# DiltheyLab/HLA-LA

Hardware: AMD Instinct MI355X
Metric: paired reads/sec aligned to PRG graph (higher is better)
Workload: dtype int32

## Files before the change

hla-la_amd/csrc/kernel_dp.hip:

```cpp
#include "batch.h"
#include "../../include/hlala_gpu.h"

namespace hlala {

enum { K_DIAG = 0, K_GGAP = 1, K_SGAP = 2, K_HOP = 3, K_JUMP = 4 };
enum { M_D = 0, M_GG = 1, M_SG = 2 };
enum { PH_IDLE = 0, PH_RUN, PH_SELECT, PH_BT, PH_EXPAND, PH_DONE };

constexpr u64 HKEY_EMPTY = ~0ull;
#ifndef HLALA_DP_PROFILE_LOG2
#define HLALA_DP_PROFILE_LOG2 18
#endif
#ifndef HLALA_EARLY_GEN_MAX
#define HLALA_EARLY_GEN_MAX 0xFFFFFE
#endif
constexpr int DP_EARLY_GEN_MAX = HLALA_EARLY_GEN_MAX;
constexpr int EXT_PENDING = 0x7FFFFFFF;
constexpr int DP_BT_STEPS_PER_TRIP = 32;

#ifndef HLALA_DP_TAIL_THREADS
#define HLALA_DP_TAIL_THREADS 128
#endif
constexpr int DP_TAIL_THREADS = HLALA_DP_TAIL_THREADS;
#ifndef HLALA_DP_TINY_WAVES
#define HLALA_DP_TINY_WAVES 4
#endif
#ifndef HLALA_DP_WIDE_THREADS
#define HLALA_DP_WIDE_THREADS 64
#endif
#ifndef HLALA_DP_BROAD_THREADS
#define HLALA_DP_BROAD_THREADS HLALA_DP_TAIL_THREADS
#endif
#ifndef HLALA_DP_LARGE_THREADS
#define HLALA_DP_LARGE_THREADS HLALA_DP_TAIL_THREADS
#endif
#ifndef HLALA_DP_HUGE_THREADS
#define HLALA_DP_HUGE_THREADS HLALA_DP_TAIL_THREADS
#endif
struct DpTiny  { static constexpr bool JF = false; static constexpr int THREADS = 64, WAVES = HLALA_DP_TINY_WAVES, GW = 16, WCAP = 16,   HC = 32,   IBITS = 4,  CELLS = 2048,     EARLY = 4096,     IMPCAP = 64,   COMPLETED = 256,          STEPS = 1024;     typedef u32 Best; typedef short Slot; typedef unsigned char ImpIdx; static constexpr bool IN_MEMORY = false; };
#ifndef HLALA_DP_TINYJF_WAVES
#define HLALA_DP_TINYJF_WAVES 4
#endif
struct DpTinyJF : DpTiny { static constexpr bool JF = true; static constexpr int WAVES = HLALA_DP_TINYJF_WAVES; };
struct DpMid   { static constexpr bool JF = false; static constexpr int THREADS = 64, WAVES = 4, GW = 32, WCAP = 32,   HC = 128,  IBITS = 5,  CELLS = 4096,     EARLY = 8192,     IMPCAP = 256,  COMPLETED = 512,          STEPS = 2048;     typedef u32 Best; typedef short Slot; typedef unsigned short ImpIdx; static constexpr bool IN_MEMORY = false; };
struct DpSmall { static constexpr bool JF = false; static constexpr int THREADS = 64, WAVES = 5, GW = 64, WCAP = 64,   HC = 128,  IBITS = 7,  CELLS = DP_CELLS, EARLY = DP_CELLS, IMPCAP = 2048, COMPLETED = DP_COMPLETED, STEPS = DP_STEPS; typedef u32 Best; typedef short Slot; typedef unsigned short ImpIdx; static constexpr bool IN_MEMORY = false; };
struct DpWide  { static constexpr bool JF = false; static constexpr int THREADS = HLALA_DP_WIDE_THREADS, WAVES = 2, GW = HLALA_DP_WIDE_THREADS, WCAP = 256,  HC = 512,  IBITS = 8,  CELLS = DP_CELLS, EARLY = DP_CELLS, IMPCAP = 2048, COMPLETED = DP_COMPLETED, STEPS = DP_STEPS; typedef u32 Best; typedef short Slot; typedef unsigned short ImpIdx; static constexpr bool IN_MEMORY = false; };
struct DpBroad { static constexpr bool JF = false; static constexpr int THREADS = HLALA_DP_BROAD_THREADS, WAVES = 1, GW = HLALA_DP_BROAD_THREADS, WCAP = 512,  HC = 1024, IBITS = 9,  CELLS = DP_CELLS_LARGE, EARLY = DP_CELLS_LARGE, IMPCAP = 4096, COMPLETED = DP_COMPLETED_LARGE, STEPS = DP_STEPS; typedef u32 Best; typedef int Slot; typedef unsigned short ImpIdx; static constexpr bool IN_MEMORY = false; };
struct DpLarge { static constexpr bool JF = false; static constexpr int THREADS = HLALA_DP_LARGE_THREADS, WAVES = 1, GW = HLALA_DP_LARGE_THREADS, WCAP = 1024, HC = 2048, IBITS = 10, CELLS = DP_CELLS_LARGE, EARLY = DP_CELLS_LARGE, IMPCAP = 4096, COMPLETED = DP_COMPLETED_LARGE, STEPS = DP_STEPS; typedef u32 Best; typedef int Slot; typedef unsigned short ImpIdx; static constexpr bool IN_MEMORY = false; };

struct DpHuge  { static constexpr bool JF = false; static constexpr int THREADS = HLALA_DP_HUGE_THREADS, WAVES = 1, GW = HLALA_DP_HUGE_THREADS, WCAP = 8192, HC = 16384, IBITS = 13, CELLS = 131072, EARLY = 131072, IMPCAP = 8192, COMPLETED = 65536, STEPS = DP_STEPS; typedef u64 Best; typedef int Slot; typedef unsigned short ImpIdx; static constexpr bool IN_MEMORY = true; };
#ifndef HLALA_DP_SORT_SCRATCH
#define HLALA_DP_SORT_SCRATCH 4096
#endif
constexpr int DP_SORT_SCRATCH = HLALA_DP_SORT_SCRATCH;

struct DpState {
    int itemIdx;
    int item, rOff, seqLen, start_seq, startLevel, startNode;
    int d, b1, b2, n1, n2, nCells, nCompleted, curMax, firstMaxSlot, lastInc, earlyInit, itersRun, diagonals;
    int earlyMaxNat;
    u32 cellsEvaluated;
    int endSlot, endScore, nSteps, nCols;
    int have, sb, se, err;
    int isAlias;
    int needTier;
};

template <bool SMALL> struct TlistT { typedef unsigned short type; };
template <> struct TlistT<true> { typedef unsigned char type; };

template <class C>
struct __align__(16) DpLdsT {
    u64 hkey[C::HC];
    typename C::Best hbest[3][C::HC];
    typename TlistT<(C::HC <= 256)>::type tlist[C::HC];
    u64 fkey[2][C::WCAP];
    typename C::Slot fslot[2][C::WCAP];
    short fD[2][C::WCAP], fG[2][C::WCAP], fS[2][C::WCAP];
    typename C::Slot tes[C::HC];
    unsigned char timp[C::HC];
    typename C::ImpIdx hq[C::HC];
    int nNew, nImp, nKeepF, err, nCompletedAdd;
    int chunkNext, chunkEnd;
    int jumpMet;
    int nTa;
    int nextPhase;
    int btSlot, btM, btX, btY, btGuard, btDone;
    DpState st;
    u64 accCalls, accIters, accCells, accEdges;
#ifdef HLALA_DP_TIMING
    long long tPh[16];
#endif
#ifdef HLALA_DP_PROFILE
    long long pfStart; int pfSlow, pfImp, pfPre, pfMaxNT, pfMaxF; long long pfPh[16];
#endif
};

struct __align__(16) CellRec { u64 key; short sc[4]; u32 bt[3]; u32 pad; };

template <class C>
struct DpSlabT {
    char* base;
    static constexpr size_t O_CELL      = 0;
    static constexpr size_t O_EARLY_KEY = O_CELL + (size_t)C::CELLS * 32;
    static constexpr size_t O_STEP_XY   = O_EARLY_KEY + (size_t)C::EARLY * 8;
    static constexpr size_t O_IMP_KEY   = O_STEP_XY + (size_t)C::STEPS * 8;
    static constexpr size_t O_IMP_NEW   = O_IMP_KEY + (size_t)C::IMPCAP * 8;
    static constexpr size_t O_IMP_BT    = O_IMP_NEW + (size_t)C::IMPCAP * 8;
    static constexpr size_t O_STEP_BT   = O_IMP_BT + (size_t)C::IMPCAP * 12;
    static constexpr size_t O_EARLY_VAL = O_STEP_BT + (size_t)C::STEPS * 4;
    static constexpr size_t O_COMPLETED = O_EARLY_VAL + (size_t)C::EARLY * 4;
    static constexpr size_t O_IMP_SLOT  = O_COMPLETED + (size_t)C::COMPLETED * 4;
    static constexpr size_t O_IMP_MASK  = O_IMP_SLOT + (size_t)C::IMPCAP * 4;
    static constexpr size_t O_TIE_SLOT  = O_IMP_MASK + (size_t)C::IMPCAP * 4;
    static constexpr size_t O_TIE_KEY   = (O_TIE_SLOT + (size_t)C::COMPLETED * 4 + 7) & ~(size_t)7;
    static constexpr size_t O_EARLY_GEN = O_TIE_KEY + (size_t)C::COMPLETED * 8;
    static constexpr size_t O_SORT_SPILL = (O_EARLY_GEN + 8 + 15) & ~(size_t)15;
    static constexpr size_t BYTES       = (O_SORT_SPILL + (C::IN_MEMORY ? (size_t)C::WCAP * 16 : 0) + 255) & ~(size_t)255;
    __device__ __forceinline__ CellRec* cell() const { return (CellRec*)(base + O_CELL); }
    __device__ __forceinline__ u64* early_key() const { return (u64*)(base + O_EARLY_KEY); }
    __device__ __forceinline__ u32* step_bt() const { return (u32*)(base + O_STEP_BT); }
    __device__ __forceinline__ u64* step_xy() const { return (u64*)(base + O_STEP_XY); }
    __device__ __forceinline__ u64* imp_key() const { return (u64*)(base + O_IMP_KEY); }
    __device__ __forceinline__ u32* imp_bt() const { return (u32*)(base + O_IMP_BT); }
    __device__ __forceinline__ short* imp_new() const { return (short*)(base + O_IMP_NEW); }
    __device__ __forceinline__ int* early_val() const { return (int*)(base + O_EARLY_VAL); }
    __device__ __forceinline__ int* completed() const { return (int*)(base + O_COMPLETED); }
    __device__ __forceinline__ int* imp_slot() const { return (int*)(base + O_IMP_SLOT); }
    __device__ __forceinline__ int* imp_mask() const { return (int*)(base + O_IMP_MASK); }
    __device__ __forceinline__ int* tie_slot() const { return (int*)(base + O_TIE_SLOT); }
    __device__ __forceinline__ u64* tie_key() const { return (u64*)(base + O_TIE_KEY); }
    __device__ __forceinline__ int* early_gen() const { return (int*)(base + O_EARLY_GEN); }
    __device__ __forceinline__ u64* sort_spill() const { return (u64*)(base + O_SORT_SPILL); }
};

template <class C>
__host__ __device__ inline size_t dp_slab_bytes() { return DpSlabT<C>::BYTES; }
template <class C>
__host__ __device__ inline size_t dp_inmemory_bytes() { return ((sizeof(DpLdsT<C>) + 255) & ~(size_t)255) + DpSlabT<C>::BYTES; }

template <int GW> __device__ __forceinline__ int grp_lane() { return (int)(threadIdx.x & (GW - 1)); }
template <int GW> __device__ __forceinline__ int grp_base() { return (int)(threadIdx.x & 63 & ~(GW - 1)); }

#define HLALA_ROW_ALLREDUCE(v, OP)                                                          \
    do {                                                                                    \
        int t_;                                                                             \
        t_ = __builtin_amdgcn_update_dpp(v, v, 0xB1, 0xF, 0xF, false); v = OP(v, t_);        \
        t_ = __builtin_amdgcn_update_dpp(v, v, 0x4E, 0xF, 0xF, false); v = OP(v, t_);        \
        t_ = __builtin_amdgcn_update_dpp(v, v, 0x141, 0xF, 0xF, false); v = OP(v, t_);           \
        t_ = __builtin_amdgcn_update_dpp(v, v, 0x140, 0xF, 0xF, false); v = OP(v, t_);                \
    } while(0)

__device__ __forceinline__ void blk_barrier()
{
    __builtin_amdgcn_fence(__ATOMIC_RELEASE, "workgroup"); __builtin_amdgcn_s_barrier(); __builtin_amdgcn_fence(__ATOMIC_ACQUIRE, "workgroup");
}
template <int GW> struct BlkX { static constexpr int NW = GW / 64; };
template <int GW> __device__ __forceinline__ int* blk_words() { __shared__ int x[BlkX<GW>::NW > 0 ? 2 * BlkX<GW>::NW : 2]; return x; }

template <int GW> __device__ __forceinline__ int grp_max_i32(int v)
{
    if(GW == 64) return wave_max_i32(v);
    if constexpr (GW > 64) {
        const int w = wave_max_i32(v); int* x = blk_words<GW>();
        if(lane_id() == 0) x[threadIdx.x >> 6] = w;
        blk_barrier();
        int r = x[0];
#pragma unroll
        for(int i = 1; i < BlkX<GW>::NW; i++) r = op_max_(r, x[i]);
        blk_barrier();
        return r;
    } else {
    HLALA_ROW_ALLREDUCE(v, op_max_);
    if(GW == 32) v = op_max_(v, __shfl_xor(v, 16));
    return v;
    }
}
template <int GW> __device__ __forceinline__ int grp_sum_i32(int v)
{
    if(GW == 64) return wave_sum_i32(v);
    if constexpr (GW > 64) {
        const int w = wave_sum_i32(v); int* x = blk_words<GW>();
        if(lane_id() == 0) x[threadIdx.x >> 6] = w;
        blk_barrier();
        int r = x[0];
#pragma unroll
        for(int i = 1; i < BlkX<GW>::NW; i++) r += x[i];
        blk_barrier();
        return r;
    } else {
    HLALA_ROW_ALLREDUCE(v, op_add_);
    if(GW == 32) v = op_add_(v, __shfl_xor(v, 16));
    return v;
    }
}
template <int GW> __device__ __forceinline__ u64 grp_min_u64(u64 v)
{
    if(GW == 64) return wave_min_u64(v);
    int hi = (int)(~(u32)(v >> 32) ^ 0x80000000u);
    int mh = grp_max_i32<GW>(hi);
    int lo = (hi == mh) ? (int)(~(u32)v ^ 0x80000000u) : (int)0x80000000;
    int ml = grp_max_i32<GW>(lo);
    return ((u64)(~((u32)mh ^ 0x80000000u)) << 32) | (u64)(~((u32)ml ^ 0x80000000u));
// ... 168 lines not shown
#pragma nounroll
    for(int probe = 0; probe < C::HC; probe++) {
        u64 old = atomicCAS(&S.hkey[h], HKEY_EMPTY, key);
        if(old == HKEY_EMPTY || old == key) { typename C::Best v; pack_best<C>(v, score, order); atomicMax(&S.hbest[mat][h], v); return true; }
        h = (h + 1) & (C::HC - 1);
    }
    return false;
}

template <class C>
__device__ inline u32 dp_probe(DpLdsT<C>& S, u64 key, u32 h)
{
#pragma nounroll
    for(int probe = 1; probe < C::HC; probe++) {
        h = (h + 1) & (C::HC - 1);
        u64 old = atomicCAS(&S.hkey[h], HKEY_EMPTY, key);
        if(old == HKEY_EMPTY || old == key) return h;
    }
    return (u32)C::HC;
}
template <class C>
__device__ inline u32 dp_probe(DpLdsT<C>& S, u64 key, u32 h, bool& claimed)
{
#pragma nounroll
    for(int probe = 1; probe < C::HC; probe++) {
        h = (h + 1) & (C::HC - 1);
        u64 old = atomicCAS(&S.hkey[h], HKEY_EMPTY, key);
        if(old == HKEY_EMPTY) claimed = true;
        if(old == HKEY_EMPTY || old == key) return h;
    }
    return (u32)C::HC;
}

template <class C> __device__ __forceinline__ u32 early_hash(u64 k) { return (C::EARLY > 8192 ? hash_mix(k) : hash64(k)) & (u32)(C::EARLY - 1); }

__device__ __forceinline__ u64 early_word(int gen, u64 key) { return ((u64)(u32)gen << 40) | (key & 0xFFFFFFFFFFull); }

template <class C>
__device__ inline int early_lookup(const DpSlabT<C>& sl, int gen, u64 key)
{
    u32 h = early_hash<C>(key);
    const u64 w = early_word(gen, key);
    for(int probe = 0; probe < C::EARLY; probe++) {
        u64 cur = __hip_atomic_load(&sl.early_key()[h], __ATOMIC_RELAXED, __HIP_MEMORY_SCOPE_AGENT);
        if(cur == w) return __hip_atomic_load(&sl.early_val()[h], __ATOMIC_RELAXED, __HIP_MEMORY_SCOPE_AGENT);
        if((int)(cur >> 40) != gen) return -1;
        h = (h + 1) & (C::EARLY - 1);
    }
    return -1;
}
template <class C>
__device__ inline bool early_insert(const DpSlabT<C>& sl, int gen, u64 key, int slot)
{
    u32 h = early_hash<C>(key);
    const u64 w = early_word(gen, key);
    for(int probe = 0; probe < C::EARLY; probe++) {
        u64 cur = __hip_atomic_load(&sl.early_key()[h], __ATOMIC_RELAXED, __HIP_MEMORY_SCOPE_AGENT);
        while((int)(cur >> 40) != gen) {
            const u64 old = atomicCAS(&sl.early_key()[h], cur, w);
            if(old == cur) { cur = w; break; }
            cur = old;
        }
        if(cur == w) { __hip_atomic_store(&sl.early_val()[h], slot, __ATOMIC_RELAXED, __HIP_MEMORY_SCOPE_AGENT); return true; }
        h = (h + 1) & (C::EARLY - 1);
    }
    return false;
}

__device__ inline int dec_len(int v) { int n = 1; while(v >= 10) { v /= 10; n++; } return n; }
__device__ inline int pow10i(int n) { int p = 1; while(n-- > 0) p *= 10; return p; }
__device__ __forceinline__ int dec_len_cmp(int v)
{
    return 1 + (v >= 10) + (v >= 100) + (v >= 1000) + (v >= 10000) + (v >= 100000) + (v >= 1000000) + (v >= 10000000) + (v >= 100000000) + (v >= 1000000000);
}
__device__ __forceinline__ u32 pow10_u32(int k)
{
    u32 p = (k & 1) ? 10u : 1u;
    if(k & 2) p *= 100u;
    if(k & 4) p *= 10000u;
    if(k & 8) p *= 100000000u;
    return p;
}
__device__ __forceinline__ int xz_part(int a, int b)
{
    if(a == b) return 0;
    const int la = dec_len_cmp(a), lb = dec_len_cmp(b);
    u64 A = (u64)(u32)a, Bv = (u64)(u32)b;
    if(la < lb) A *= (u64)pow10_u32(lb - la); else if(lb < la) Bv *= (u64)pow10_u32(la - lb);
    if(A != Bv) return A < Bv ? -1 : 1;
    return la < lb ? -1 : 1;
}
__device__ __forceinline__ bool xz_less(int x1, int z1, int x2, int z2)
{
    const int c = xz_part(x1, x2);
    if(c) return c < 0;
    return xz_part(z1, z2) < 0;
}

__device__ inline u64 xz_key(int x, int z)
{
    const int lx = dec_len(x), lz = dec_len(z);
    u64 k = 0; int n = 0;
    for(int i = 0; i < lx; i++, n++) k = k * 12 + (u64)(2 + (x / pow10i(lx - 1 - i)) % 10);
    k = k * 12 + 1; n++;
    for(int i = 0; i < lz && n < 14; i++, n++) k = k * 12 + (u64)(2 + (z / pow10i(lz - 1 - i)) % 10);
    for(; n < 14; n++) k *= 12;
    return k;
}

struct __align__(16) DpItem { int item, rOff, seqLen, start_seq, startLevel, startNode, pad0, pad1; };

#ifndef HLALA_DP_SIDE_TIER
#define HLALA_DP_SIDE_TIER 3
#endif
constexpr int DP_SIDE_TIER = HLALA_DP_SIDE_TIER;
constexpr int DP_LAST_TIER = 6;
constexpr int DP_POOL_TIER = DP_SIDE_TIER > 4 ? DP_SIDE_TIER : 4;
constexpr int DP_POOL_MAX = 8;
__device__ __forceinline__ int tier_for_frontier(int n) { return n <= DpMid::WCAP ? 1 : (n <= DpSmall::WCAP ? 2 : (n <= DpWide::WCAP ? 3 : (n <= DpBroad::WCAP ? 4 : (n <= DpLarge::WCAP ? 5 : 6)))); }
__device__ __forceinline__ int tier_for_targets(int n) { return n <= (DpMid::HC * 3) / 4 ? 1 : (n <= (DpSmall::HC * 3) / 4 ? 2 : (n <= (DpWide::HC * 3) / 4 ? 3 : (n <= (DpBroad::HC * 3) / 4 ? 4 : (n <= (DpLarge::HC * 3) / 4 ? 5 : 6)))); }

#define DP_FAIL(code) do { if(gl == 0 && S.err == 0) S.err = (code); } while(0)

template <class C, class DG>
__device__ inline int dp_begin(DpLdsT<C>& S, const DpSlabT<C>& sl, const DG& G, const DpItem& it, int itemIdx)
{
    constexpr int GW = C::GW;
    const int gl = grp_lane<GW>();
    for(int i = gl; i < C::HC; i += GW) { S.hkey[i] = HKEY_EMPTY; S.hbest[0][i] = 0; S.hbest[1][i] = 0; S.hbest[2][i] = 0; }
    if(gl == 0) {
        DpState& st = S.st;
        st.itemIdx = itemIdx;
        st.item = it.item; st.rOff = it.rOff; st.seqLen = it.seqLen; st.start_seq = it.start_seq; st.startLevel = it.startLevel; st.startNode = it.startNode;
        st.diagonals = it.seqLen + G.L - 1;
        st.d = 1; st.b1 = 0; st.b2 = 1; st.n1 = 1; st.n2 = 0; st.nCells = 1; st.nCompleted = 0;
        st.curMax = 0; st.firstMaxSlot = 0; st.lastInc = 0; st.earlyInit = 0; st.earlyMaxNat = -1; st.itersRun = 0;
        st.cellsEvaluated = 0;
        st.endSlot = -1; st.endScore = 0; st.nSteps = 0; st.nCols = 0;
        st.have = 0; st.sb = 0; st.se = -1; st.err = 0; st.needTier = 0; st.isAlias = 0;
        S.err = 0; S.nTa = 0; S.jumpMet = 0;
#ifdef HLALA_DP_PROFILE
        S.pfStart = clock64(); S.pfSlow = 0; S.pfImp = 0; S.pfPre = 0; S.pfMaxNT = 0; S.pfMaxF = 0; for(int i = 0; i < 16; i++) S.pfPh[i] = 0;
#endif
        CellRec c0; c0.key = mk_key(it.startLevel, it.start_seq, it.startNode);
        c0.sc[0] = 0; c0.sc[1] = (short)DP_NEG; c0.sc[2] = (short)DP_NEG; c0.sc[3] = 0; c0.bt[0] = 0; c0.bt[1] = 0; c0.bt[2] = 0; c0.pad = 0;
        sl.cell()[0] = c0;
        S.fkey[0][0] = mk_key(it.startLevel, it.start_seq, it.startNode); S.fslot[0][0] = 0;
        S.fD[0][0] = 0; S.fG[0][0] = (short)DP_NEG; S.fS[0][0] = (short)DP_NEG;
    }
    DSYNC();
    return PH_RUN;
}

template <class C, class DG>
__device__ inline int dp_iterate(DpLdsT<C>& S, const DpSlabT<C>& sl, const DG& G, const int4* nrec, const uint8_t* readBases, const bool fwd, int& edgesAcc, u64* sortScratch)
{
    constexpr int GW = C::GW;
    const int gl = grp_lane<GW>();
    DpState& st = S.st;
    const int dir = fwd ? 1 : -1;
    const int seqLen = guni<GW>(st.seqLen);
    const int max_levelI = G.L - 1, max_seqI = seqLen;
    const int limitY = fwd ? seqLen : 0;
    const int d = guni<GW>(st.d);
    const int n1 = guni<GW>(st.n1), n2 = guni<GW>(st.n2);
    const int b1 = guni<GW>(st.b1), b2 = guni<GW>(st.b2), bn = b2;
    const int lastInc0 = guni<GW>(st.lastInc), diagonals = guni<GW>(st.diagonals);
    const uint8_t* seqp = readBases + guni<GW>(st.rOff);

    if(d > diagonals || (d - lastInc0) > 40) return PH_SELECT;
    if(n1 == 0 && n2 == 0) {
        int last = lastInc0 + 40; if(last > diagonals) last = diagonals;
        if(gl == 0) st.itersRun = last;
        DSYNC();
        return PH_SELECT;
    }
    if(d > 60000) { if(gl == 0) { st.itersRun = d; st.err = __LINE__; } DSYNC(); return PH_DONE; }

#if defined(HLALA_DP_TIMING)
    long long tq0 = clock64();
#define DP_TQ(i) do { __builtin_amdgcn_s_waitcnt(0); long long t_ = clock64(); if(gl == 0) S.tPh[i] += t_ - tq0; tq0 = t_; } while(0)
#elif defined(HLALA_DP_PROFILE)
    long long tq0 = clock64();
#define DP_TQ(i) do { __builtin_amdgcn_s_waitcnt(0); long long t_ = clock64(); if(gl == 0) S.pfPh[i] += t_ - tq0; tq0 = t_; } while(0)
#else
#define DP_TQ(i) do { } while(0)
#endif
    const int* eoff = fwd ? G.out_off : G.in_off; const int* eto = fwd ? G.out_to : G.in_from; const uint8_t* elab = fwd ? G.out_label : G.in_label;
    const int* joff = fwd ? G.jf_off : G.jb_off; const int* jnode = fwd ? G.jf_node : G.jb_node; const int* jlvl = fwd ? G.jf_lvl : G.jb_lvl;
    const uint8_t* eprk = fwd ? G.out_prank : G.in_prank; const uint8_t* jprk = fwd ? G.jf_prank : G.jb_prank;
    int edges = 0;
    const int nMax = n1 > n2 ? n1 : n2;
    constexpr bool APPEND = (GW >= 64) && (C::WCAP > 64);
    typedef typename TlistT<(C::HC <= 256)>::type TlT;
    int nTa = 0;
    auto append = [&](const bool claimed, const u32 h) {
        if constexpr (APPEND && GW == 64) {
            const u64 m = __ballot(claimed);
            if(claimed) S.tlist[nTa + (int)__builtin_amdgcn_mbcnt_hi((u32)(m >> 32), __builtin_amdgcn_mbcnt_lo((u32)m, 0u))] = (TlT)h;
            nTa += __popcll(m);
        } else if constexpr (APPEND) {
            const u64 m = __ballot(claimed);
            if(m) {
                int base = 0;
                if(lane_id() == 0) base = atomicAdd(&S.nTa, (int)__popcll(m));
                base = __builtin_amdgcn_readfirstlane(base);
                const int pos = base + (int)__builtin_amdgcn_mbcnt_hi((u32)(m >> 32), __builtin_amdgcn_mbcnt_lo((u32)m, 0u));
                if(claimed && pos < C::HC) S.tlist[pos] = (TlT)h;
            }
        }
    };
    for(int i = gl; i < nMax; i += GW) {
        const bool hasA = i < n2, hasB = i < n1;
        u64 pkA = hasA ? S.fkey[b2][i] : 0, pkB = hasB ? S.fkey[b1][i] : 0;
        const int pxA = key_x(pkA), pyA = key_y(pkA), nodeA = key_node(pkA);
        const int pxB = key_x(pkB), pyB = key_y(pkB), nodeB = key_node(pkB);
        const int nxA = pxA + dir, nyA = pyA + dir;
        const bool doA = hasA && !(nxA > max_levelI || nyA > max_seqI || nxA < 0 || nyA < 0);
        const int pDA = hasA ? (int)S.fD[b2][i] : 0;
        const int pD = hasB ? (int)S.fD[b1][i] : 0, pG = hasB ? (int)S.fG[b1][i] : 0, pS = hasB ? (int)S.fS[b1][i] : 0;
        int4 ra0 = make_int4(0, 0, 0, 0), ra1 = ra0, rb0 = ra0, rb1 = ra0; unsigned char rc = 0;
        if(doA) { ra0 = nrec[2 * (size_t)nodeA]; ra1 = nrec[2 * (size_t)nodeA + 1]; rc = fwd ? seqp[pyA] : seqp[pyA - 1]; }
        if(hasB) { rb0 = nrec[2 * (size_t)nodeB]; rb1 = nrec[2 * (size_t)nodeB + 1]; }
        const int a0 = ra0.x, degA = ra0.y & 0xFFFF, tnA0 = ra0.z, tnA1 = ra0.w;
        const unsigned char labA0 = (unsigned char)(ra1.w & 0xFF), labA1 = (unsigned char)((ra1.w >> 8) & 0xFF);
        const int rkA1 = (ra1.w >> 16) & 1, rkB1 = (rb1.w >> 16) & 1;
        const int e0 = rb0.x, degB = rb0.y & 0xFFFF, tnB0 = rb0.z, tnB1 = rb0.w;
        const int j0 = rb1.x, j1 = j0 + (int)((u32)rb0.y >> 16), jn0 = rb1.y, jx0 = rb1.z;
        const unsigned char labB0 = (unsigned char)(rb1.w & 0xFF), labB1 = (unsigned char)((rb1.w >> 8) & 0xFF);
        DP_TQ(4);
        const int ord0 = (1 << (C::IBITS + 8)) | (i << 8);
        const int nyG = pyB + dir, nxB = pxB + dir;
        const bool okA = doA, okB = hasB;
        const bool sgB = okB && nxB >= 0 && nxB <= max_levelI;
        typedef typename C::Best BestT;
        {
            bool cv[3]; u64 ck[3]; u32 ch[3]; u64 cold[3];
            cv[0] = okA && degA > 0; ck[0] = mk_key(nxA, nyA, tnA0);
            cv[1] = okA && degA > 1; ck[1] = mk_key(nxA, nyA, tnA1);
            cv[2] = hasB && nyG >= 0 && nyG <= max_seqI; ck[2] = mk_key(pxB, nyG, nodeB);
#pragma unroll
            for(int q = 0; q < 3; q++) { ch[q] = tgt_hash<C>(ck[q]); cold[q] = HKEY_EMPTY; if(cv[q]) cold[q] = atomicCAS(&S.hkey[ch[q]], HKEY_EMPTY, ck[q]); }
            if constexpr (APPEND) {
                bool cl[3];
#pragma unroll
                for(int q = 0; q < 3; q++) {
                    cl[q] = cv[q] && cold[q] == HKEY_EMPTY;
                    if(cv[q] && !(cold[q] == HKEY_EMPTY || cold[q] == ck[q])) { ch[q] = dp_probe<C>(S, ck[q], ch[q], cl[q]); if(ch[q] >= (u32)C::HC) { S.err = __LINE__; cv[q] = false; cl[q] = false; } }
                }
#pragma unroll
                for(int q = 0; q < 3; q++) append(cl[q], ch[q]);
            } else {
#pragma unroll
                for(int q = 0; q < 3; q++)
                    if(cv[q] && !(cold[q] == HKEY_EMPTY || cold[q] == ck[q])) { ch[q] = dp_probe<C>(S, ck[q], ch[q]); if(ch[q] >= (u32)C::HC) { S.err = __LINE__; cv[q] = false; } }
            }
            if(cv[0]) { BestT v; pack_best<C>(v, pDA + (labA0 == rc ? 2 : -5), (i << 8) | 0); atomicMax(&S.hbest[M_D][ch[0]], v); }
            if(cv[1]) { BestT v; pack_best<C>(v, pDA + (labA1 == rc ? 2 : -5), (i << 8) | rkA1); atomicMax(&S.hbest[M_D][ch[1]], v); }
            if(cv[2]) { BestT v, w; pack_best<C>(v, pD - 6, ord0 | 0); if(pG != DP_NEG) { pack_best<C>(w, pG - 2, ord0 | 1); if(w > v) v = w; } atomicMax(&S.hbest[M_GG][ch[2]], v); }
        }
        {
            bool cv[3]; u64 ck[3]; u32 ch[3]; u64 cold[3];
            cv[0] = sgB && degB > 0; ck[0] = mk_key(nxB, pyB, tnB0);
            cv[1] = sgB && degB > 1; ck[1] = mk_key(nxB, pyB, tnB1);
            if constexpr (C::JF) { cv[2] = false; ck[2] = 0; if(okB && j1 > j0) { S.err = __LINE__; S.jumpMet = 1; } }
            else { cv[2] = okB && j1 > j0 && jx0 >= 0 && jx0 <= max_levelI; ck[2] = mk_key(jx0, pyB, jn0); }
#pragma unroll
            for(int q = 0; q < 3; q++) { ch[q] = tgt_hash<C>(ck[q]); cold[q] = HKEY_EMPTY; if(cv[q]) cold[q] = atomicCAS(&S.hkey[ch[q]], HKEY_EMPTY, ck[q]); }
            if constexpr (APPEND) {
                bool cl[3];
#pragma unroll
                for(int q = 0; q < 3; q++) {
                    cl[q] = cv[q] && cold[q] == HKEY_EMPTY;
                    if(cv[q] && !(cold[q] == HKEY_EMPTY || cold[q] == ck[q])) { ch[q] = dp_probe<C>(S, ck[q], ch[q], cl[q]); if(ch[q] >= (u32)C::HC) { S.err = __LINE__; cv[q] = false; cl[q] = false; } }
                }
#pragma unroll
                for(int q = 0; q < 3; q++) append(cl[q], ch[q]);
            } else {
#pragma unroll
                for(int q = 0; q < 3; q++)
                    if(cv[q] && !(cold[q] == HKEY_EMPTY || cold[q] == ck[q])) { ch[q] = dp_probe<C>(S, ck[q], ch[q]); if(ch[q] >= (u32)C::HC) { S.err = __LINE__; cv[q] = false; } }
            }
#pragma unroll
            for(int kk = 0; kk < 2; kk++) {
                const unsigned char lab = kk ? labB1 : labB0;
                const int rk = kk ? rkB1 : 0;
                if(cv[kk]) {
                    BestT v, w;
                    if(lab != '_') {
                        pack_best<C>(v, pD - 6, ord0 | (2 * rk)); if(pS != DP_NEG) { pack_best<C>(w, pS - 2, ord0 | (2 * rk + 1)); if(w > v) v = w; }
                        atomicMax(&S.hbest[M_SG][ch[kk]], v);
                    } else {
                        if(pS != DP_NEG) { pack_best<C>(w, pS, ord0 | (2 * rk + 1)); atomicMax(&S.hbest[M_SG][ch[kk]], w); }
                        pack_best<C>(v, pD, ord0 | rk); atomicMax(&S.hbest[M_D][ch[kk]], v);
                    }
                }
            }
            if constexpr (!C::JF) if(cv[2]) { BestT v; pack_best<C>(v, pD, ord0 | 128); atomicMax(&S.hbest[M_D][ch[2]], v); }
        }
        if(okA) edges += degA;
        if(sgB) edges += degB;
        if constexpr (APPEND) {
            for(int k = 2; __ballot(okA && k < degA) != 0; k++) {
                int at = -1;
                if(okA && k < degA) {
                    int tn = eto[a0 + k]; unsigned char lab = elab[a0 + k];
                    if(!dp_push<C>(S, mk_key(nxA, nyA, tn), M_D, pDA + (lab == rc ? 2 : -5), (i << 8) | (int)eprk[a0 + k], at)) S.err = __LINE__;
                }
                append(at >= 0, (u32)at);
            }
            for(int kk = 2; __ballot(sgB && kk < degB) != 0; kk++) {
                int at = -1;
                if(sgB && kk < degB) {
                    int tn = eto[e0 + kk]; unsigned char lab = elab[e0 + kk]; const int rk = (int)eprk[e0 + kk];
                    u64 k = mk_key(nxB, pyB, tn);
                    if(lab != '_') {
                        if(!dp_push<C>(S, k, M_SG, pD - 6, ord0 | (2 * rk), at)) S.err = __LINE__;
                        if(pS != DP_NEG) if(!dp_push<C>(S, k, M_SG, pS - 2, ord0 | (2 * rk + 1), at)) S.err = __LINE__;
                    } else {
                        if(pS != DP_NEG) if(!dp_push<C>(S, k, M_SG, pS, ord0 | (2 * rk + 1), at)) S.err = __LINE__;
                        if(!dp_push<C>(S, k, M_D, pD, ord0 | rk, at)) S.err = __LINE__;
                    }
                }
                append(at >= 0, (u32)at);
            }
            for(int j = j0 + 1; __ballot(okB && j < j1) != 0; j++) {
                int at = -1;
                if(okB && j < j1) {
                    int tn = jnode[j]; int jx = jlvl[j];
                    if(!(jx < 0 || jx > max_levelI)) if(!dp_push<C>(S, mk_key(jx, pyB, tn), M_D, pD, ord0 | (128 + (int)jprk[j]), at)) S.err = __LINE__;
                }
                append(at >= 0, (u32)at);
            }
        } else {
            if(okA) for(int k = 2; k < degA; k++) {
                int tn = eto[a0 + k]; unsigned char lab = elab[a0 + k];
                if(!dp_push<C>(S, mk_key(nxA, nyA, tn), M_D, pDA + (lab == rc ? 2 : -5), (i << 8) | (int)eprk[a0 + k])) S.err = __LINE__;
            }
            if(sgB) for(int kk = 2; kk < degB; kk++) {
                int tn = eto[e0 + kk]; unsigned char lab = elab[e0 + kk]; const int rk = (int)eprk[e0 + kk];
                u64 k = mk_key(nxB, pyB, tn);
                if(lab != '_') {
                    if(!dp_push<C>(S, k, M_SG, pD - 6, ord0 | (2 * rk))) S.err = __LINE__;
                    if(pS != DP_NEG) if(!dp_push<C>(S, k, M_SG, pS - 2, ord0 | (2 * rk + 1))) S.err = __LINE__;
                } else {
                    if(pS != DP_NEG) if(!dp_push<C>(S, k, M_SG, pS, ord0 | (2 * rk + 1))) S.err = __LINE__;
                    if(!dp_push<C>(S, k, M_D, pD, ord0 | rk)) S.err = __LINE__;
                }
            }
            if constexpr (!C::JF) if(okB) for(int j = j0 + 1; j < j1; j++) {
                int tn = jnode[j]; int jx = jlvl[j];
                if(jx < 0 || jx > max_levelI) continue;
                if(!dp_push<C>(S, mk_key(jx, pyB, tn), M_D, pD, ord0 | (128 + (int)jprk[j]))) S.err = __LINE__;
            }
        }
    }
    edgesAcc += edges;
    DSYNC();
    DP_TQ(5);
    int nT = 0;
    if constexpr (APPEND && GW == 64) nT = __builtin_amdgcn_readfirstlane(nTa);
    else if constexpr (APPEND) { nT = guni<GW>(S.nTa); if(nT > C::HC) nT = C::HC + 1; }
    else if constexpr (C::IN_MEMORY) {
        for(int h0 = 0; h0 < C::HC; h0 += 4 * GW) {
            u64 kk[4];
#pragma unroll
            for(int q = 0; q < 4; q++) kk[q] = __hip_atomic_load(&S.hkey[h0 + q * GW + gl], __ATOMIC_RELAXED, __HIP_MEMORY_SCOPE_AGENT);
#pragma unroll
            for(int q = 0; q < 4; q++) {
                const bool occ = kk[q] != HKEY_EMPTY;
                int tot; const int rk = grp_rank<GW>(occ, tot);
                if(occ) S.tlist[nT + rk] = (typename TlistT<(C::HC <= 256)>::type)(h0 + q * GW + gl);
                nT += tot;
            }
        }
    } else
    for(int h0 = 0; h0 < C::HC; h0 += GW) {
        const int h = h0 + gl;
        const bool occ = S.hkey[h] != HKEY_EMPTY;
        int tot; const int rk = grp_rank<GW>(occ, tot);
        if(occ) S.tlist[nT + rk] = (typename TlistT<(C::HC <= 256)>::type)h;
        nT += tot;
    }
    DSYNC();
    DP_TQ(0);
    if(nT > (C::HC * 3) / 4 || guni<GW>(S.err)) { if(gl == 0) { st.itersRun = d; st.err = __LINE__; if(nT > (C::HC * 3) / 4) st.needTier = tier_for_targets(nT); } DSYNC(); return PH_DONE; }

    const int startLevel = guni<GW>(st.startLevel), start_seq = guni<GW>(st.start_seq);
    const int curMax0 = guni<GW>(st.curMax);
    const int nCompleted0 = guni<GW>(st.nCompleted);
    int nCells = guni<GW>(st.nCells);
    int earlyInit = guni<GW>(st.earlyInit);
    const int earlyMaxNat0 = guni<GW>(st.earlyMaxNat);
    if(gl == 0) { S.nNew = 0; S.nImp = 0; S.nCompletedAdd = 0; S.nTa = 0; }
    DSYNC();
    int itMaxNew = DP_NEG;
    u64 itMaxKey = ~0ull;
    bool anyEqDiff = false, anyOw = false, anyExisting = false;

    const bool prepass = !C::JF && earlyInit && d <= earlyMaxNat0;
    int earlyNatMax = -1;
    if(prepass) {
        for(int t0 = 0; t0 < nT; t0 += GW) {
            int t = t0 + gl; int es = -1;
            if(t < nT) {
                int h = S.tlist[t];
                int Dv = max(best_score<C>(S.hbest[M_D][h]), max(best_score<C>(S.hbest[M_GG][h]), best_score<C>(S.hbest[M_SG][h])));
                if(Dv >= -16) es = early_lookup<C>(sl, earlyInit, S.hkey[h]);
                S.tes[t] = (typename C::Slot)es;
            }
            if(es >= 0) anyExisting = true;
        }
        anyExisting = grp_any<GW>(anyExisting);
        DSYNC();
    }
    DP_TQ(3);
    const bool slow = anyExisting;
    const bool hadEarly = prepass;
    bool failed = false;

    for(int pass = 0; pass < (slow ? 2 : 1); pass++) {
        for(int t0 = 0; t0 < nT; t0 += GW) {
            int t = t0 + gl;
            bool act = t < nT;
            int h = act ? S.tlist[t] : 0;
            u64 key = act ? S.hkey[h] : 0;
            typename C::Best bD = act ? S.hbest[M_D][h] : 0, bG = act ? S.hbest[M_GG][h] : 0, bS = act ? S.hbest[M_SG][h] : 0;
            int Dc = best_score<C>(bD), GGv = best_score<C>(bG), SGv = best_score<C>(bS);
            int Dv = Dc, dsel = 0;
            if(GGv > Dv) { Dv = GGv; dsel = 1; }
            if(SGv > Dv) { Dv = SGv; dsel = 2; }
            bool keep = act && (Dv >= -16);
            DP_TQ(8);
            int es = -1; bool isNew; int slot;
            if(pass == 0) {
                if(hadEarly && act) S.hq[h] = (typename C::ImpIdx)~0u;
                if(hadEarly && keep) { int v = S.tes[t]; if(v >= 0) es = v; }
                isNew = keep && es < 0;
                int total; int off = grp_excl_scan<GW>(isNew ? 1 : 0, total);
                slot = isNew ? nCells + off : es;
                if(nCells + total > C::CELLS) { DP_FAIL(__LINE__); failed = true; }
                nCells += total;
            } else {
                slot = keep ? S.tes[t] : -1;
                isNew = keep && (S.timp[t] & 0x80);
                es = isNew ? -1 : slot;
            }
            const bool ok = !failed && S.err == 0;
            DP_TQ(9);
            u32 btD = 0, btG = 0, btS = 0;
            int srcScore = 0;
            if(keep && ok && slot >= 0 && slot < C::CELLS) {
                if(bG) { int o = best_order<C>(bG); int i = (o >> 8) & ((1 << C::IBITS) - 1); int j = o & 255;
                         btG = mk_bt(S.fslot[b1][i], j ? 1 : 0, K_GGAP, -1); }
                if(bS) { int o = best_order<C>(bS); int i = (o >> 8) & ((1 << C::IBITS) - 1); int j = o & 255;
                         btS = mk_bt(S.fslot[b1][i], (j & 1) ? 2 : 0, K_SGAP, j >> 1); }
                if(dsel == 0) {
                    int o = best_order<C>(bD); int ph = o >> (C::IBITS + 8); int i = (o >> 8) & ((1 << C::IBITS) - 1); int j = o & 255;
                    int sb = ph ? b1 : b2;
                    srcScore = S.fD[sb][i];
                    if(!ph) btD = mk_bt(S.fslot[sb][i], 0, K_DIAG, j);
                    else if(j < 128) btD = mk_bt(S.fslot[sb][i], 0, K_SGAP, j);
                    else btD = mk_bt(S.fslot[sb][i], 0, K_JUMP, j - 128);
                } else if(dsel == 1) {
                    btD = mk_bt(slot, 1, K_HOP, -1);
                    int o = best_order<C>(bG); int i = (o >> 8) & ((1 << C::IBITS) - 1); int j = o & 255;
                    srcScore = j ? S.fG[b1][i] : S.fD[b1][i];
                } else {
                    btD = mk_bt(slot, 2, K_HOP, -1);
                    int o = best_order<C>(bS); int i = (o >> 8) & ((1 << C::IBITS) - 1); int j = o & 255;
                    srcScore = (j & 1) ? S.fS[b1][i] : S.fD[b1][i];
                }
            }
            DP_TQ(10);
            int impMask = 0;
            int mD = Dv, mG = GGv, mS = SGv;
            u32 mbtD = btD;
            if(pass == 0) {
                if(isNew && ok && slot < C::CELLS) {
                    uint4* dst = (uint4*)(sl.cell() + slot);
                    dst[0] = make_uint4((u32)key, (u32)(key >> 32), ((u32)(unsigned short)(short)Dv) | ((u32)(unsigned short)(short)GGv << 16), (u32)(unsigned short)(short)SGv);
                    dst[1] = make_uint4(btD, btG, btS, 0u);
                }
                int x = key_x(key), y = key_y(key);
                int natural = (x > startLevel ? x - startLevel : startLevel - x) + (y > start_seq ? y - start_seq : start_seq - y);
                bool isEarly = !C::JF && isNew && natural > d;
                if(isEarly && natural > earlyNatMax) earlyNatMax = natural;
                if(grp_any<GW>(isEarly)) {
                    if(!earlyInit) {
                        int g = 0;
                        if(gl == 0) g = __hip_atomic_load(sl.early_gen(), __ATOMIC_RELAXED, __HIP_MEMORY_SCOPE_AGENT) + 1;
                        g = grp_bcast0<GW>(g);
                        if(g > DP_EARLY_GEN_MAX) { for(int i = gl; i < C::EARLY; i += GW) sl.early_key()[i] = 0; g = 1; }
                        if(gl == 0) __hip_atomic_store(sl.early_gen(), g, __ATOMIC_RELAXED, __HIP_MEMORY_SCOPE_AGENT);
                        earlyInit = g;
                        DSYNC();
                    }
                    if(isEarly) if(!early_insert<C>(sl, earlyInit, key, slot)) S.err = __LINE__;
                }
                if(isNew && y == limitY) {
                    int pos = atomicAdd(&S.nCompletedAdd, 1);
                    if(nCompleted0 + pos < C::COMPLETED) sl.completed()[nCompleted0 + pos] = slot; else S.err = __LINE__;
                }
            }
            DP_TQ(11);
            if constexpr (!C::JF) if(keep && !isNew && ok) {
// ... 909 lines not shown
```

Measured before the change: 5.731 million.

## Batch node-record and base loads via inline asm, unroll edge expansion loads

Replaces the per-lane int4 node-record loads and the read-base byte load with one inline-asm group that issues every global load at once under an exec mask and waits a single time. It also batches the edge, jump-target loads (EDGE_BATCH of 4 for wide configs) so several loads are in flight before the hash pushes. An empty asm barrier forces the jump loads to issue before the range test. The aim is to cut serialized global memory latency in the diagonal expansion loop. The cost is more register pressure and fragile hand-written asm: the non-JF path rebuilds parts of the second record from partial loads, and the second loads always run, even for lanes without B.

```diff
diff --git a/hla-la_amd/csrc/kernel_dp.hip b/hla-la_amd/csrc/kernel_dp.hip
--- a/hla-la_amd/csrc/kernel_dp.hip
+++ b/hla-la_amd/csrc/kernel_dp.hip
@@ -37,18 +37,18 @@
 #ifndef HLALA_DP_HUGE_THREADS
 #define HLALA_DP_HUGE_THREADS HLALA_DP_TAIL_THREADS
 #endif
-struct DpTiny  { static constexpr bool JF = false; static constexpr int THREADS = 64, WAVES = HLALA_DP_TINY_WAVES, GW = 16, WCAP = 16,   HC = 32,   IBITS = 4,  CELLS = 2048,     EARLY = 4096,     IMPCAP = 64,   COMPLETED = 256,          STEPS = 1024;     typedef u32 Best; typedef short Slot; typedef unsigned char ImpIdx; static constexpr bool IN_MEMORY = false; };
+struct DpTiny  { static constexpr bool JF = false, REC_BATCH = true; static constexpr int EDGE_BATCH = 1; static constexpr int THREADS = 64, WAVES = HLALA_DP_TINY_WAVES, GW = 16, WCAP = 16,   HC = 32,   IBITS = 4,  CELLS = 2048,     EARLY = 4096,     IMPCAP = 64,   COMPLETED = 256,          STEPS = 1024;     typedef u32 Best; typedef short Slot; typedef unsigned char ImpIdx; static constexpr bool IN_MEMORY = false; };
 #ifndef HLALA_DP_TINYJF_WAVES
 #define HLALA_DP_TINYJF_WAVES 4
 #endif
 struct DpTinyJF : DpTiny { static constexpr bool JF = true; static constexpr int WAVES = HLALA_DP_TINYJF_WAVES; };
-struct DpMid   { static constexpr bool JF = false; static constexpr int THREADS = 64, WAVES = 4, GW = 32, WCAP = 32,   HC = 128,  IBITS = 5,  CELLS = 4096,     EARLY = 8192,     IMPCAP = 256,  COMPLETED = 512,          STEPS = 2048;     typedef u32 Best; typedef short Slot; typedef unsigned short ImpIdx; static constexpr bool IN_MEMORY = false; };
-struct DpSmall { static constexpr bool JF = false; static constexpr int THREADS = 64, WAVES = 5, GW = 64, WCAP = 64,   HC = 128,  IBITS = 7,  CELLS = DP_CELLS, EARLY = DP_CELLS, IMPCAP = 2048, COMPLETED = DP_COMPLETED, STEPS = DP_STEPS; typedef u32 Best; typedef short Slot; typedef unsigned short ImpIdx; static constexpr bool IN_MEMORY = false; };
-struct DpWide  { static constexpr bool JF = false; static constexpr int THREADS = HLALA_DP_WIDE_THREADS, WAVES = 2, GW = HLALA_DP_WIDE_THREADS, WCAP = 256,  HC = 512,  IBITS = 8,  CELLS = DP_CELLS, EARLY = DP_CELLS, IMPCAP = 2048, COMPLETED = DP_COMPLETED, STEPS = DP_STEPS; typedef u32 Best; typedef short Slot; typedef unsigned short ImpIdx; static constexpr bool IN_MEMORY = false; };
-struct DpBroad { static constexpr bool JF = false; static constexpr int THREADS = HLALA_DP_BROAD_THREADS, WAVES = 1, GW = HLALA_DP_BROAD_THREADS, WCAP = 512,  HC = 1024, IBITS = 9,  CELLS = DP_CELLS_LARGE, EARLY = DP_CELLS_LARGE, IMPCAP = 4096, COMPLETED = DP_COMPLETED_LARGE, STEPS = DP_STEPS; typedef u32 Best; typedef int Slot; typedef unsigned short ImpIdx; static constexpr bool IN_MEMORY = false; };
-struct DpLarge { static constexpr bool JF = false; static constexpr int THREADS = HLALA_DP_LARGE_THREADS, WAVES = 1, GW = HLALA_DP_LARGE_THREADS, WCAP = 1024, HC = 2048, IBITS = 10, CELLS = DP_CELLS_LARGE, EARLY = DP_CELLS_LARGE, IMPCAP = 4096, COMPLETED = DP_COMPLETED_LARGE, STEPS = DP_STEPS; typedef u32 Best; typedef int Slot; typedef unsigned short ImpIdx; static constexpr bool IN_MEMORY = false; };
-
-struct DpHuge  { static constexpr bool JF = false; static constexpr int THREADS = HLALA_DP_HUGE_THREADS, WAVES = 1, GW = HLALA_DP_HUGE_THREADS, WCAP = 8192, HC = 16384, IBITS = 13, CELLS = 131072, EARLY = 131072, IMPCAP = 8192, COMPLETED = 65536, STEPS = DP_STEPS; typedef u64 Best; typedef int Slot; typedef unsigned short ImpIdx; static constexpr bool IN_MEMORY = true; };
+struct DpMid   { static constexpr bool JF = false, REC_BATCH = true; static constexpr int EDGE_BATCH = 1; static constexpr int THREADS = 64, WAVES = 4, GW = 32, WCAP = 32,   HC = 128,  IBITS = 5,  CELLS = 4096,     EARLY = 8192,     IMPCAP = 256,  COMPLETED = 512,          STEPS = 2048;     typedef u32 Best; typedef short Slot; typedef unsigned short ImpIdx; static constexpr bool IN_MEMORY = false; };
+struct DpSmall { static constexpr bool JF = false, REC_BATCH = true; static constexpr int EDGE_BATCH = 1; static constexpr int THREADS = 64, WAVES = 5, GW = 64, WCAP = 64,   HC = 128,  IBITS = 7,  CELLS = DP_CELLS, EARLY = DP_CELLS, IMPCAP = 2048, COMPLETED = DP_COMPLETED, STEPS = DP_STEPS; typedef u32 Best; typedef short Slot; typedef unsigned short ImpIdx; static constexpr bool IN_MEMORY = false; };
+struct DpWide  { static constexpr bool JF = false, REC_BATCH = true; static constexpr int EDGE_BATCH = 4; static constexpr int THREADS = HLALA_DP_WIDE_THREADS, WAVES = 2, GW = HLALA_DP_WIDE_THREADS, WCAP = 256,  HC = 512,  IBITS = 8,  CELLS = DP_CELLS, EARLY = DP_CELLS, IMPCAP = 2048, COMPLETED = DP_COMPLETED, STEPS = DP_STEPS; typedef u32 Best; typedef short Slot; typedef unsigned short ImpIdx; static constexpr bool IN_MEMORY = false; };
+struct DpBroad { static constexpr bool JF = false, REC_BATCH = true; static constexpr int EDGE_BATCH = 4; static constexpr int THREADS = HLALA_DP_BROAD_THREADS, WAVES = 1, GW = HLALA_DP_BROAD_THREADS, WCAP = 512,  HC = 1024, IBITS = 9,  CELLS = DP_CELLS_LARGE, EARLY = DP_CELLS_LARGE, IMPCAP = 4096, COMPLETED = DP_COMPLETED_LARGE, STEPS = DP_STEPS; typedef u32 Best; typedef int Slot; typedef unsigned short ImpIdx; static constexpr bool IN_MEMORY = false; };
+struct DpLarge { static constexpr bool JF = false, REC_BATCH = true; static constexpr int EDGE_BATCH = 4; static constexpr int THREADS = HLALA_DP_LARGE_THREADS, WAVES = 1, GW = HLALA_DP_LARGE_THREADS, WCAP = 1024, HC = 2048, IBITS = 10, CELLS = DP_CELLS_LARGE, EARLY = DP_CELLS_LARGE, IMPCAP = 4096, COMPLETED = DP_COMPLETED_LARGE, STEPS = DP_STEPS; typedef u32 Best; typedef int Slot; typedef unsigned short ImpIdx; static constexpr bool IN_MEMORY = false; };
+
+struct DpHuge  { static constexpr bool JF = false, REC_BATCH = true; static constexpr int EDGE_BATCH = 4; static constexpr int THREADS = HLALA_DP_HUGE_THREADS, WAVES = 1, GW = HLALA_DP_HUGE_THREADS, WCAP = 8192, HC = 16384, IBITS = 13, CELLS = 131072, EARLY = 131072, IMPCAP = 8192, COMPLETED = 65536, STEPS = DP_STEPS; typedef u64 Best; typedef int Slot; typedef unsigned short ImpIdx; static constexpr bool IN_MEMORY = true; };
 #ifndef HLALA_DP_SORT_SCRATCH
 #define HLALA_DP_SORT_SCRATCH 4096
 #endif
@@ -523,6 +523,43 @@
     return PH_RUN;
 }
 
+typedef int dp_i32x4 __attribute__((ext_vector_type(4)));
+typedef int dp_i32x2 __attribute__((ext_vector_type(2)));
+__device__ __forceinline__ void dp_load_round(u64& qa, u64& qb, const uint8_t* bases, const u32 chOff, const u64 chMask, dp_i32x4& ra0, dp_i32x4& rb0, dp_i32x2& rb1xy, u32& rc)
+{
+    u64 ex;
+    asm volatile("global_load_dwordx4 %0, %4, off\n\t"
+                 "global_load_dwordx4 %1, %5, off\n\t"
+                 "global_load_dwordx2 %2, %5, off offset:16\n\t"
+                 "global_load_dwordx2 %4, %4, off offset:24\n\t"
+                 "global_load_dwordx2 %5, %5, off offset:24\n\t"
+                 "s_mov_b64 %6, exec\n\t"
+                 "s_and_b64 exec, exec, %9\n\t"
+                 "global_load_ubyte %3, %7, %8\n\t"
+                 "s_mov_b64 exec, %6\n\t"
+                 "s_waitcnt vmcnt(0)"
+                 : "=&v"(ra0), "=&v"(rb0), "=&v"(rb1xy), "=v"(rc), "+v"(qa), "+v"(qb), "=&s"(ex)
+                 : "v"(chOff), "s"(bases), "s"(chMask)
+                 : "scc");
+}
+__device__ __forceinline__ void dp_keep_loaded(int& a, int& b, int& c) { asm volatile("" : "+v"(a), "+v"(b), "+v"(c)); }
+__device__ __forceinline__ void dp_load_round_jf(const u64 qa, const u64 qb, const uint8_t* bases, const u32 chOff, const u64 chMask, dp_i32x4& ra0, dp_i32x4& rb0, u32& wa, u32& wb, u32& rc)
+{
+    u64 ex;
+    asm volatile("global_load_dwordx4 %0, %6, off\n\t"
+                 "global_load_dwordx4 %1, %7, off\n\t"
+                 "global_load_dword %3, %6, off offset:28\n\t"
+                 "global_load_dword %4, %7, off offset:28\n\t"
+                 "s_mov_b64 %5, exec\n\t"
+                 "s_and_b64 exec, exec, %10\n\t"
+                 "global_load_ubyte %2, %8, %9\n\t"
+                 "s_mov_b64 exec, %5\n\t"
+                 "s_waitcnt vmcnt(0)"
+                 : "=&v"(ra0), "=&v"(rb0), "=v"(rc), "=&v"(wa), "=&v"(wb), "=&s"(ex)
+                 : "v"(qa), "v"(qb), "v"(chOff), "s"(bases), "s"(chMask)
+                 : "scc");
+}
+
 template <class C, class DG>
 __device__ inline int dp_iterate(DpLdsT<C>& S, const DpSlabT<C>& sl, const DG& G, const int4* nrec, const uint8_t* readBases, const bool fwd, int& edgesAcc, u64* sortScratch)
 {
@@ -537,7 +574,8 @@
     const int n1 = guni<GW>(st.n1), n2 = guni<GW>(st.n2);
     const int b1 = guni<GW>(st.b1), b2 = guni<GW>(st.b2), bn = b2;
     const int lastInc0 = guni<GW>(st.lastInc), diagonals = guni<GW>(st.diagonals);
-    const uint8_t* seqp = readBases + guni<GW>(st.rOff);
+    const int rOff = guni<GW>(st.rOff);
+    const uint8_t* seqp = readBases + rOff;
 
     if(d > diagonals || (d - lastInc0) > 40) return PH_SELECT;
     if(n1 == 0 && n2 == 0) {
@@ -591,8 +629,19 @@
         const int pDA = hasA ? (int)S.fD[b2][i] : 0;
         const int pD = hasB ? (int)S.fD[b1][i] : 0, pG = hasB ? (int)S.fG[b1][i] : 0, pS = hasB ? (int)S.fS[b1][i] : 0;
         int4 ra0 = make_int4(0, 0, 0, 0), ra1 = ra0, rb0 = ra0, rb1 = ra0; unsigned char rc = 0;
-        if(doA) { ra0 = nrec[2 * (size_t)nodeA]; ra1 = nrec[2 * (size_t)nodeA + 1]; rc = fwd ? seqp[pyA] : seqp[pyA - 1]; }
-        if(hasB) { rb0 = nrec[2 * (size_t)nodeB]; rb1 = nrec[2 * (size_t)nodeB + 1]; }
+        if constexpr (C::REC_BATCH) {
+            const u32 chOff = (u32)(rOff + (fwd ? pyA : pyA - 1));
+            u32 rcw;
+            u64 qa = (u64)(nrec + 2 * (size_t)nodeA), qb = (u64)(nrec + 2 * (size_t)nodeB);
+            dp_i32x4 a, b;
+            if constexpr (C::JF) { u32 wa, wb; dp_load_round_jf(qa, qb, readBases, chOff, __ballot(doA), a, b, wa, wb, rcw); ra1.w = (int)wa; rb1.w = (int)wb; }
+            else { dp_i32x2 xy; dp_load_round(qa, qb, readBases, chOff, __ballot(doA), a, b, xy, rcw); rb1.x = xy.x; rb1.y = xy.y; rb1.z = (int)(u32)qb; ra1.w = (int)(qa >> 32); rb1.w = (int)(qb >> 32); }
+            ra0 = make_int4(a.x, a.y, a.z, a.w); rb0 = make_int4(b.x, b.y, b.z, b.w);
+            rc = (unsigned char)rcw;
+        } else {
+            if(doA) { ra0 = nrec[2 * (size_t)nodeA]; ra1 = nrec[2 * (size_t)nodeA + 1]; rc = fwd ? seqp[pyA] : seqp[pyA - 1]; }
+            if(hasB) { rb0 = nrec[2 * (size_t)nodeB]; rb1 = nrec[2 * (size_t)nodeB + 1]; }
+        }
         const int a0 = ra0.x, degA = ra0.y & 0xFFFF, tnA0 = ra0.z, tnA1 = ra0.w;
         const unsigned char labA0 = (unsigned char)(ra1.w & 0xFF), labA1 = (unsigned char)((ra1.w >> 8) & 0xFF);
         const int rkA1 = (ra1.w >> 16) & 1, rkB1 = (rb1.w >> 16) & 1;
@@ -671,37 +720,74 @@
         }
         if(okA) edges += degA;
         if(sgB) edges += degB;
-        if constexpr (APPEND) {
-            for(int k = 2; __ballot(okA && k < degA) != 0; k++) {
-                int at = -1;
+        constexpr int EB = C::EDGE_BATCH;
+        auto more = [](const bool p) { if constexpr (APPEND) return __ballot(p) != 0; else return p; };
+        auto push = [&](const u64 key, const int mat, const int score, const int order, int& at) {
+            if constexpr (APPEND) return dp_push<C>(S, key, mat, score, order, at); else return dp_push<C>(S, key, mat, score, order);
+        };
+        static_assert(EB >= 1, "EDGE_BATCH");
+        if constexpr (APPEND || EB > 1) {
+            for(int k = 2; more(okA && k < degA); k += EB) {
+                int at[EB];
+#pragma unroll
+                for(int q = 0; q < EB; q++) at[q] = -1;
                 if(okA && k < degA) {
-                    int tn = eto[a0 + k]; unsigned char lab = elab[a0 + k];
-                    if(!dp_push<C>(S, mk_key(nxA, nyA, tn), M_D, pDA + (lab == rc ? 2 : -5), (i << 8) | (int)eprk[a0 + k], at)) S.err = __LINE__;
-                }
-                append(at >= 0, (u32)at);
-            }
-            for(int kk = 2; __ballot(sgB && kk < degB) != 0; kk++) {
-                int at = -1;
+                    int tn[EB]; unsigned char lab[EB], rk[EB];
+#pragma unroll
+                    for(int q = 0; q < EB; q++) { const int e = a0 + (EB > 1 ? min(k + q, degA - 1) : k); tn[q] = eto[e]; lab[q] = elab[e]; rk[q] = eprk[e]; }
+#pragma unroll
+                    for(int q = 0; q < EB; q++)
+                        if(k + q < degA) if(!push(mk_key(nxA, nyA, tn[q]), M_D, pDA + (lab[q] == rc ? 2 : -5), (i << 8) | (int)rk[q], at[q])) S.err = __LINE__;
+                }
+                if constexpr (APPEND) {
+#pragma unroll
+                    for(int q = 0; q < EB; q++) append(at[q] >= 0, (u32)at[q]);
+                }
+            }
+            for(int kk = 2; more(sgB && kk < degB); kk += EB) {
+                int at[EB];
+#pragma unroll
+                for(int q = 0; q < EB; q++) at[q] = -1;
                 if(sgB && kk < degB) {
-                    int tn = eto[e0 + kk]; unsigned char lab = elab[e0 + kk]; const int rk = (int)eprk[e0 + kk];
-                    u64 k = mk_key(nxB, pyB, tn);
-                    if(lab != '_') {
-                        if(!dp_push<C>(S, k, M_SG, pD - 6, ord0 | (2 * rk), at)) S.err = __LINE__;
-                        if(pS != DP_NEG) if(!dp_push<C>(S, k, M_SG, pS - 2, ord0 | (2 * rk + 1), at)) S.err = __LINE__;
-                    } else {
-                        if(pS != DP_NEG) if(!dp_push<C>(S, k, M_SG, pS, ord0 | (2 * rk + 1), at)) S.err = __LINE__;
-                        if(!dp_push<C>(S, k, M_D, pD, ord0 | rk, at)) S.err = __LINE__;
+                    int tn[EB]; unsigned char lab[EB], rkk[EB];
+#pragma unroll
+                    for(int q = 0; q < EB; q++) { const int e = e0 + (EB > 1 ? min(kk + q, degB - 1) : kk); tn[q] = eto[e]; lab[q] = elab[e]; rkk[q] = eprk[e]; }
+#pragma unroll
+                    for(int q = 0; q < EB; q++) if(kk + q < degB) {
+                        const int rk = (int)rkk[q];
+                        const u64 k = mk_key(nxB, pyB, tn[q]);
+                        if(lab[q] != '_') {
+                            if(!push(k, M_SG, pD - 6, ord0 | (2 * rk), at[q])) S.err = __LINE__;
+                            if(pS != DP_NEG) if(!push(k, M_SG, pS - 2, ord0 | (2 * rk + 1), at[q])) S.err = __LINE__;
+                        } else {
+                            if(pS != DP_NEG) if(!push(k, M_SG, pS, ord0 | (2 * rk + 1), at[q])) S.err = __LINE__;
+                            if(!push(k, M_D, pD, ord0 | rk, at[q])) S.err = __LINE__;
+                        }
                     }
                 }
-                append(at >= 0, (u32)at);
-            }
-            for(int j = j0 + 1; __ballot(okB && j < j1) != 0; j++) {
-                int at = -1;
+                if constexpr (APPEND) {
+#pragma unroll
+                    for(int q = 0; q < EB; q++) append(at[q] >= 0, (u32)at[q]);
+                }
+            }
+            if constexpr (!C::JF) for(int j = j0 + 1; more(okB && j < j1); j += EB) {
+                int at[EB];
+#pragma unroll
+                for(int q = 0; q < EB; q++) at[q] = -1;
                 if(okB && j < j1) {
-                    int tn = jnode[j]; int jx = jlvl[j];
-                    if(!(jx < 0 || jx > max_levelI)) if(!dp_push<C>(S, mk_key(jx, pyB, tn), M_D, pD, ord0 | (128 + (int)jprk[j]), at)) S.err = __LINE__;
-                }
-                append(at >= 0, (u32)at);
+                    int tn[EB], jx[EB], rk[EB];
+#pragma unroll
+                    for(int q = 0; q < EB; q++) { const int e = EB > 1 ? min(j + q, j1 - 1) : j; tn[q] = jnode[e]; jx[q] = jlvl[e]; rk[q] = (int)jprk[e]; }
+#pragma unroll
+                    for(int q = 0; q < EB; q++) dp_keep_loaded(tn[q], jx[q], rk[q]);
+#pragma unroll
+                    for(int q = 0; q < EB; q++)
+                        if(j + q < j1 && !(jx[q] < 0 || jx[q] > max_levelI)) if(!push(mk_key(jx[q], pyB, tn[q]), M_D, pD, ord0 | (128 + rk[q]), at[q])) S.err = __LINE__;
+                }
+                if constexpr (APPEND) {
+#pragma unroll
+                    for(int q = 0; q < EB; q++) append(at[q] >= 0, (u32)at[q]);
+                }
             }
         } else {
             if(okA) for(int k = 2; k < degA; k++) {
@@ -720,9 +806,10 @@
                 }
             }
             if constexpr (!C::JF) if(okB) for(int j = j0 + 1; j < j1; j++) {
-                int tn = jnode[j]; int jx = jlvl[j];
+                int tn = jnode[j]; int jx = jlvl[j]; int rk = (int)jprk[j];
+                dp_keep_loaded(tn, jx, rk);
                 if(jx < 0 || jx > max_levelI) continue;
-                if(!dp_push<C>(S, mk_key(jx, pyB, tn), M_D, pD, ord0 | (128 + (int)jprk[j]))) S.err = __LINE__;
+                if(!dp_push<C>(S, mk_key(jx, pyB, tn), M_D, pD, ord0 | (128 + rk))) S.err = __LINE__;
             }
         }
     }
```

Result: no change. 5.758 million, median of 6 (+0.5%).
